# openai/multiagent-particle-envs

Measured on AMD Instinct MI355X. Metric: env steps/sec (whole node), simple_spread N=3, batch=65536 per GPU, higher is better.
Workload: dtype f32; 1 GPU; simple_spread A=3 L=3, 65536 worlds/GPU, fresh one-hot moves, reset every 25 steps; steps commanded to the step server; protocol=fresh, step-server (one doorbell per episode), batch_per_gpu=65536, global_batch=65536, mode=step-server, commands=auto, barrier_backend=none

## Files before the change

### multiagent_particle_envs_amd/csrc/mpe_split.hip

```cpp
#include <type_traits>

#include "mpe_internal.h"

#ifndef MPE_SPLIT_ABLATE
#define MPE_SPLIT_ABLATE 0
#endif

#ifdef MPE_PHASE_CLOCK
#define MPE_STAMP(k)                                                                                              \
  do {                                                                                                            \
    if (blockIdx.x < 4 && lane == 0 && b.force && t < 32)                                                         \
      reinterpret_cast<unsigned long long *>(b.force)[(((size_t)blockIdx.x * 16 + role) * 32 + t) * 8 + (k)] =     \
          __builtin_amdgcn_s_memtime();                                                                           \
  } while (0)
#else
#define MPE_STAMP(k) do { } while (0)
#endif

#ifdef MPE_DEVICE_SPAN
#define MPE_SPAN_BEGIN() const unsigned long long span_t0_ = (unsigned long long)wall_clock64()
#define MPE_SPAN_END()                                                                                             \
  do {                                                                                                             \
    if (b_in.force && (threadIdx.x & 63) == 0 && (threadIdx.x >> 6) < 8) {                                           \
      const uintptr_t sp_ = reinterpret_cast<uintptr_t>(b_in.force);                                                \
      if (sp_ & 1) asm volatile("s_waitcnt vmcnt(0) lgkmcnt(0)" ::: "memory");                                      \
      ulonglong2 st_;                                                                                              \
      st_.x = span_t0_;                                                                                            \
      st_.y = (unsigned long long)wall_clock64();                                                                  \
      reinterpret_cast<ulonglong2 *>(sp_ & ~(uintptr_t)7)[(size_t)blockIdx.x * 8 + (threadIdx.x >> 6)] = st_;       \
    }                                                                                                              \
  } while (0)
#else
#define MPE_SPAN_BEGIN() do { } while (0)
#define MPE_SPAN_END() do { } while (0)
#endif

namespace mpe {

#ifndef MPE_SPLIT_DUAL
#define MPE_SPLIT_DUAL 1
#endif
#ifndef MPE_SPLIT_DUAL_OWN_DRAW
#define MPE_SPLIT_DUAL_OWN_DRAW (1 << MPE_SCN_SPREAD)
#endif
template <int KIND>
constexpr bool dual_own_draw() { return ((MPE_SPLIT_DUAL_OWN_DRAW) >> KIND) & 1; }

template <int KIND>
constexpr bool dual_kind() {
  return (MPE_SPLIT_DUAL) &&
         (KIND == MPE_SCN_SIMPLE || KIND == MPE_SCN_SPREAD || KIND == MPE_SCN_TAG || KIND == MPE_SCN_ADVERSARY || KIND == MPE_SCN_PUSH);
}

template <int KIND, int A, int L, int NADV>
struct SplitShape {
  static constexpr int E = A + L;
  static constexpr int XW = KIND == MPE_SCN_SPREAD ? 4 + L
                            : (KIND == MPE_SCN_SIMPLE || KIND == MPE_SCN_ADVERSARY || KIND == MPE_SCN_PUSH ||
                               KIND == MPE_SCN_SPEAKER_LISTENER || KIND == MPE_SCN_REFERENCE) ? 5
                            : KIND == MPE_SCN_WORLD_COMM ? 6 : 4;
  static constexpr int DC = KIND == MPE_SCN_SPEAKER_LISTENER ? 3 : KIND == MPE_SCN_REFERENCE ? 10
                            : (KIND == MPE_SCN_CRYPTO || KIND == MPE_SCN_WORLD_COMM) ? 4 : 2;
  static constexpr int NCH = (KIND == MPE_SCN_ADVERSARY || KIND == MPE_SCN_PUSH || KIND == MPE_SCN_SPEAKER_LISTENER) ? 1
                             : (KIND == MPE_SCN_REFERENCE || KIND == MPE_SCN_CRYPTO) ? 2 : 0;
  static constexpr int DMAX = KIND == MPE_SCN_SIMPLE   ? 2 + 2 * L
                              : KIND == MPE_SCN_SPREAD ? 4 + 2 * L + 4 * (A - 1)
                              : KIND == MPE_SCN_TAG    ? 4 + 2 * L + 2 * (A - 1) + 2 * (A - NADV)
                              : KIND == MPE_SCN_ADVERSARY ? 2 + 2 * L + 2 * (A - 1)
                              : KIND == MPE_SCN_PUSH   ? 7 + 5 * L + 2 * (A - 1)
                              : KIND == MPE_SCN_SPEAKER_LISTENER ? 2 + 2 * L + 3
                              : KIND == MPE_SCN_REFERENCE ? 2 + 2 * L + 3 + 10
                              : KIND == MPE_SCN_CRYPTO ? 8
                              : KIND == MPE_SCN_WORLD_COMM ? 4 + 2 * L + 2 * (A - 1) + 2 * (A - NADV) + 2 + 4
                                                       : 1;
  static constexpr int trows(bool roll) { return (KIND == MPE_SCN_WORLD_COMM && roll) ? 32 : kWave; }
  static constexpr int tile_floats(bool roll) { return trows(roll) * (DMAX | 1); }
  static constexpr int waves(bool dual) { return (dual ? 2 * A : A) + 1; }
  static constexpr size_t lds_bytes(bool roll) {
    return sizeof(float) * ((roll ? 2 : 1) * A * XW * kWave + A * tile_floats(roll) + (roll ? 2 * A * kWave : 0));
  }
};

template <int KIND>
constexpr unsigned speakers_of() {
  return KIND == MPE_SCN_SPEAKER_LISTENER ? 0x1u : KIND == MPE_SCN_REFERENCE ? 0x3u : KIND == MPE_SCN_CRYPTO ? 0x7u
         : KIND == MPE_SCN_WORLD_COMM ? 0x1u : 0u;
}
constexpr int kWordRow = 0, kWordDrawn = 1, kWordRowSys = 2;
template <int WM>
struct Word {
  const float *row;
  int id;
  __device__ __forceinline__ float operator[](int c) const {
    if constexpr (WM == kWordDrawn) return c == id ? 1.f : 0.f;
    else if constexpr (WM == kWordRowSys)
      return __builtin_bit_cast(float, __hip_atomic_load(reinterpret_cast<const int *>(row) + c, __ATOMIC_RELAXED, __HIP_MEMORY_SCOPE_SYSTEM));
    else return row[c];
  }
};
template <int DC, int WM>
__device__ __forceinline__ Word<WM> word_of(const MpeBuffers &b, size_t B, size_t w0, unsigned ln, int j, uint64_t seed,
                                            uint64_t gw, uint64_t gt) {
  Word<WM> wd;
  wd.row = WM == kWordDrawn ? nullptr : b.comm + wave_off(((size_t)j * B + w0) * DC) + ln * DC;
  wd.id = WM == kWordDrawn ? comm_draw(seed, gw, gt, j, DC) : 0;
  return wd;
}

template <int KIND, int RP>
constexpr int aux_policy() { return (KIND == MPE_SCN_TAG && RP == kRowsSc1) ? kRowsSc1 : kRowsPlain; }

template <int KIND, int A, int L, int NADV, bool ROLL, int AUX, int WM = (ROLL ? kWordDrawn : kWordRow)>
__device__ __forceinline__ void reward_wave(const NarrowDesc &d, const float *const sz , const MpeBuffers &b, const float *X, int lane,
                                            bool live, unsigned ln, size_t B, size_t w0 ,
                                            size_t ro , uint64_t seed, uint64_t gw,
                                            uint64_t gt, int goal_roll ,
                                            const float (&food_roll)[4] ) {
  constexpr int XW = SplitShape<KIND, A, L, NADV>::XW;
  if (KIND == MPE_SCN_SIMPLE) {
    if (live) {
#pragma unroll
      for (int a = 0; a < A; ++a) {
        if (b.rew) store_aux<AUX>(b.rew + wave_off(ro + (size_t)a * B) + ln, -X[(a * XW + 4) * kWave + lane]);
        if (b.done) store_aux<AUX>(b.done + wave_off(ro + (size_t)a * B) + ln, 0);
      }
    }
  }
  if (KIND == MPE_SCN_SPREAD) {
    if (b.rew || b.info_rew) {
      float px[A], py[A];
#pragma unroll
      for (int a = 0; a < A; ++a) {
        px[a] = X[(a * XW + 0) * kWave + lane];
        py[a] = X[(a * XW + 1) * kWave + lane];
      }
      float lm_term = 0.f, md = 0.f;
      int occupied = 0;
#pragma unroll
      for (int l = 0; l < L; ++l) {
        float m2 = X[(0 * XW + 4 + l) * kWave + lane];
#pragma unroll
        for (int a = 1; a < A; ++a) m2 = fminf(m2, X[(a * XW + 4 + l) * kWave + lane]);
        const float m = fast_sqrt(m2);
        lm_term = lm_term - m;
        md = md + m;
        if (b.info_rew) occupied += sqrt_lt(m2, 0.1f) ? 1 : 0;
      }
      int cnt[A];
#pragma unroll
      for (int a = 0; a < A; ++a) cnt[a] = (sz[a] + sz[a] > 0.f) ? 1 : 0;
#pragma unroll
      for (int a = 0; a < A; ++a) {
#pragma unroll
        for (int c = a + 1; c < A; ++c) {
          const bool hit = sqrt_lt(sq2d(px[a] - px[c], py[a] - py[c]), sz[a] + sz[c]);
          cnt[a] += hit ? 1 : 0;
          cnt[c] += hit ? 1 : 0;
        }
      }
      float r[A];
#pragma unroll
      for (int a = 0; a < A; ++a) {
        const int c = ((d.collide >> a) & 1u) ? cnt[a] : 0;
        cnt[a] = c;
        float ra_ = lm_term;
#pragma unroll
        for (int s = 0; s < A; ++s) ra_ = ra_ - (c > s ? 1.f : 0.f);
        r[a] = ra_;
      }
// ... 157 lines not shown
    for (int g = 0; g < NG; ++g)
#pragma unroll
      for (int v = 0; v < NADV; ++v) {
        const float d2 = sq2d(px[NADV + g] - px[v], py[NADV + g] - py[v]);
        hit[g][v] = sqrt_lt(d2, sz[NADV + g] + sz[v]);
        dmin[v] = fminf(dmin[v], d2);
      }
    float fx[2], fy[2];
#pragma unroll
    for (int f = 0; f < 2; ++f) {
      fx[f] = ROLL ? food_roll[2 * f] : (b.pos + wave_off((size_t)(2 * (A + 1 + f)) * B + w0))[ln];
      fy[f] = ROLL ? food_roll[2 * f + 1] : (b.pos + wave_off((size_t)(2 * (A + 1 + f) + 1) * B + w0))[ln];
    }
    if (live) {
#pragma unroll
      for (int a = 0; a < A; ++a) {
        float r = 0.f;
        if (a < NADV) {
          r = r - 0.1f * fast_sqrt(dmin[a < NADV ? a : 0]);
          if ((d.collide >> a) & 1u) {
#pragma unroll
            for (int g = 0; g < NG; ++g)
#pragma unroll
              for (int v = 0; v < NADV; ++v) r = r + (hit[g][v] ? 5.f : 0.f);
          }
        } else {
          if ((d.collide >> a) & 1u) {
#pragma unroll
            for (int v = 0; v < NADV; ++v) r = r - (hit[a >= NADV ? a - NADV : 0][v] ? 5.f : 0.f);
          }
          r = r - 2.f * tag_bound(fabsf(px[a]));
          r = r - 2.f * tag_bound(fabsf(py[a]));
          float m2 = INFINITY;
#pragma unroll
          for (int f = 0; f < 2; ++f) {
            const float d2 = sq2d(px[a] - fx[f], py[a] - fy[f]);
            r = r + (sqrt_lt(d2, sz[a] + sz[A + 1 + f]) ? 2.f : 0.f);
            m2 = fminf(m2, d2);
          }
          r = r + 0.05f * fast_sqrt(m2);
        }
        const size_t o = ro + (size_t)a * B;
        if (b.rew) store_aux<AUX>(b.rew + wave_off(o) + ln, r);
        if (b.done) store_aux<AUX>(b.done + wave_off(o) + ln, 0);
        if (b.info_collisions) {
          int c = 0;
          if (a < NADV) {
#pragma unroll
            for (int g = 0; g < NG; ++g) c += hit[g][a < NADV ? a : 0] ? 1 : 0;
          }
          store_aux<AUX>(b.info_collisions + wave_off(o) + ln, c);
        }
      }
    }
  }
}

typedef float vf2 __attribute__((ext_vector_type(2)));
typedef __attribute__((address_space(4))) const vf2 cvf2;
__device__ __forceinline__ vf2 pol_act2(vf2 x, bool tnh) { return vf2{pol_act(x.x, tnh), pol_act(x.y, tnh)}; }
template <int NO2>
__device__ __forceinline__ void pol_layer0(const cvf2 *W, const float *row, int sw, int D, float *rec, vf2 (&h)[NO2]) {
#pragma unroll
  for (int j = 0; j < NO2; ++j) h[j] = W[D * NO2 + j];
  for (int k = 0; k < D; ++k) {
    const float x = row[(((k >> 2) ^ sw) << 2) | (k & 3)];
    if (rec) rec[k] = x;
    const vf2 xx = {x, x};
#pragma unroll
    for (int j = 0; j < NO2; ++j) h[j] = __builtin_elementwise_fma(W[k * NO2 + j], xx, h[j]);
  }
}
template <int NO2>
__device__ __forceinline__ void pol_layer(const cvf2 *W, const vf2 (&h)[32], vf2 (&o)[NO2]) {
#pragma unroll
  for (int j = 0; j < NO2; ++j) o[j] = W[64 * NO2 + j];
#pragma unroll
  for (int k = 0; k < 64; ++k) {
    const float x = (k & 1) ? h[k >> 1].y : h[k >> 1].x;
    const vf2 xx = {x, x};
#pragma unroll
    for (int j = 0; j < NO2; ++j) o[j] = __builtin_elementwise_fma(W[k * NO2 + j], xx, o[j]);
    if ((k & 3) == 3) __builtin_amdgcn_sched_barrier(0);
  }
}
__device__ __forceinline__ void pol_logits(const float *Wg, int nl, bool tnh, const float *row, int sw, int D, float *rec,
                                           float (&z)[5]) {
  const cvf2 *W = (const cvf2 *)(uintptr_t)Wg;
  vf2 o[4];
  if (nl == 1) {
    pol_layer0<4>(W, row, sw, D, rec, o);
  } else {
    vf2 h[32];
    pol_layer0<32>(W, row, sw, D, rec, h);
#pragma unroll
    for (int j = 0; j < 32; ++j) h[j] = pol_act2(h[j], tnh);
    const cvf2 *W1 = W + (size_t)(D + 1) * 32;
    if (nl == 2) {
      pol_layer<4>(W1, h, o);
    } else {
      const cvf2 *W2 = W1 + 65 * 32;
#pragma unroll
      for (int j = 0; j < 4; ++j) o[j] = W2[64 * 4 + j];
#pragma unroll 1
      for (int c = 0; c < 4; ++c) {
        vf2 g[8];
#pragma unroll
        for (int j = 0; j < 8; ++j) g[j] = W1[64 * 32 + 8 * c + j];
#pragma unroll
        for (int k = 0; k < 64; ++k) {
          const float x = (k & 1) ? h[k >> 1].y : h[k >> 1].x;
          const vf2 xx = {x, x};
#pragma unroll
          for (int j = 0; j < 8; ++j) g[j] = __builtin_elementwise_fma(W1[k * 32 + 8 * c + j], xx, g[j]);
          if ((k & 7) == 7) __builtin_amdgcn_sched_barrier(0);
        }
#pragma unroll
        for (int u = 0; u < 16; ++u) {
          const float x = pol_act((u & 1) ? g[u >> 1].y : g[u >> 1].x, tnh);
          const vf2 xx = {x, x};
#pragma unroll
          for (int j = 0; j < 4; ++j) o[j] = __builtin_elementwise_fma(W2[(16 * c + u) * 4 + j], xx, o[j]);
        }
      }
    }
  }
  z[0] = o[0].x; z[1] = o[0].y; z[2] = o[1].x; z[3] = o[1].y; z[4] = o[2].x;
}

template <int AUX>
__device__ __forceinline__ void store_state(const MpeBuffers &b, size_t B, int i, size_t w0, unsigned ln, float mx,
                                            float my, float mvx, float mvy) {
  store_aux<AUX>(b.pos + wave_off((size_t)(2 * i) * B + w0) + ln, mx);
  store_aux<AUX>(b.pos + wave_off((size_t)(2 * i + 1) * B + w0) + ln, my);
  store_aux<AUX>(b.vel + wave_off((size_t)(2 * i) * B + w0) + ln, mvx);
  store_aux<AUX>(b.vel + wave_off((size_t)(2 * i + 1) * B + w0) + ln, mvy);
}

struct ServeArgs {
  unsigned long long *door;
  unsigned long long *flag;
  unsigned int *status;
  const float *act_ring;
  const float *comm_ring;
  int32_t ring, slots;
  unsigned long long timeout_ticks;
};
__device__ __forceinline__ unsigned long long door_load(const unsigned long long *p) {
  const unsigned long long v = __hip_atomic_load(p, __ATOMIC_RELAXED, __HIP_MEMORY_SCOPE_SYSTEM);
  const uint32_t lo = __builtin_amdgcn_readfirstlane((uint32_t)v), hi = __builtin_amdgcn_readfirstlane((uint32_t)(v >> 32));
  return ((unsigned long long)hi << 32) | lo;
}
__device__ __forceinline__ void drain_stores() { asm volatile("s_waitcnt vmcnt(0)" ::: "memory"); }

template <int KIND, int A, int L, int NADV, bool ROLL, int RP ,
          bool DUALP = false ,
          bool SERVE = false ,
          bool POL = false >
__device__ __forceinline__ void split_body(float *const g_pos, float *const g_vel, const float *const g_act, const int32_t *const g_ids,
                                           const size_t B, const int g_wpw, const int g_observe_only, const unsigned g_movable,
                                           const NarrowDesc &d, const MpeBuffers &b_in, const RollArgs &ra, const ServeArgs &sv,
                                           const PolArgs &pol) {
  static_assert(!SERVE || (ROLL && RP == kRowsSc1), "the step server: a rollout instantiation, write-through stores");
  static_assert(!POL || (ROLL && !SERVE && !DUALP), "the policy rollout: a single-role rollout instantiation");
  static_assert(!POL || KIND == MPE_SCN_SIMPLE || KIND == MPE_SCN_SPREAD || KIND == MPE_SCN_ADVERSARY || KIND == MPE_SCN_PUSH,
                "the policy rollout: scenarios whose observation rows read no other agent's velocity");
  constexpr int WM = SERVE ? kWordRowSys : (ROLL ? kWordDrawn : kWordRow);
  using S = SplitShape<KIND, A, L, NADV>;
  MPE_SPAN_BEGIN();
  MpeBuffers b = b_in;
  b.pos = g_pos;
  b.vel = g_vel;
  b.act = g_act;
  b.ids = g_ids;
  constexpr int E = A + L, XW = S::XW;
  constexpr int AUX = SERVE ? kRowsSc1 : aux_policy<KIND, RP>();
  extern __shared__ __attribute__((aligned(16))) float smem[];
  const int lane = threadIdx.x & (kWave - 1);
  constexpr bool DUAL = DUALP && ROLL;
  constexpr bool OWN_DRAW = DUAL && dual_own_draw<KIND>();
  constexpr int NAW = DUAL ? 2 * A : A;
  const int role = __builtin_amdgcn_readfirstlane((int)(threadIdx.x >> 6));
  const bool is_agent = role < NAW;
  const bool is_rows = DUAL && role >= A && role < NAW;
  const int i = is_agent ? (role >= A ? role - A : role) : 0;
  const int wpw = g_wpw;
  const size_t w0 = (size_t)blockIdx.x * (size_t)wpw;
  if (w0 >= B) return;
#ifdef MPE_STRESS_DELAY_WAVE
  if (role == (MPE_STRESS_DELAY_WAVE) % A)
    for (int k = 0; k < 10; ++k) __builtin_amdgcn_s_sleep(127);
#endif
  const int nvalid = (B - w0) < (size_t)wpw ? (int)(B - w0) : wpw;
  const bool live = lane < nvalid;
  const unsigned ln = (unsigned)(live ? lane : nvalid - 1) & 63u;
  const size_t w = w0 + (size_t)ln;
  float *const xch = smem;
  float *const tile = smem + (ROLL ? 2 : 1) * A * XW * kWave + i * S::tile_floats(ROLL);
  int *const mv = reinterpret_cast<int *>(smem + (ROLL ? 2 : 1) * A * XW * kWave + A * S::tile_floats(ROLL));

  const int T = ROLL ? ra.T : 1;
  const size_t obs_stride = (ra.trajectory || SERVE) ? (size_t)d.obs_off[A] * B : 0;
  const size_t row_stride = (ra.trajectory || SERVE) ? (size_t)A * B : 0;
  int blk0 = 0, mvt0 = 0;
  unsigned long long seen = 0;
  int *const idle_cnt = reinterpret_cast<int *>(smem + SplitShape<KIND, A, L, NADV>::lds_bytes(true) / sizeof(float));
  if constexpr (SERVE) {
    blk0 = (int)(ra.step0 % (uint64_t)sv.slots);
    mvt0 = (int)(ra.step0 % (uint64_t)sv.ring);
    if (threadIdx.x < 3) idle_cnt[threadIdx.x] = 0;
    __syncthreads();
  }
  auto block_of = [&](const int t) { return SERVE ? (blk0 + t) % sv.slots : t; };
  auto with_words = [&](const int t) {
    MpeBuffers q = b;
    if constexpr (SERVE)
      q.comm = sv.comm_ring ? sv.comm_ring + (size_t)((mvt0 + t) % sv.ring) * ((size_t)A * B * SplitShape<KIND, A, L, NADV>::DC) : nullptr;
    return q;
  };
  auto wait_door = [&](const int t, const bool publisher) -> bool {
    if constexpr (!SERVE) return true;
    const unsigned long long g = ra.step0 + (unsigned long long)t;
    if (seen > g) return true;
    seen = door_load(sv.door);
    if (seen > g) return true;
    drain_stores();
    bool told = t == 0;
    if (!publisher && !told && lane == 0) __hip_atomic_fetch_add(&idle_cnt[t & 1], 1, __ATOMIC_RELEASE, __HIP_MEMORY_SCOPE_WORKGROUP);
    const unsigned long long t_begin = (unsigned long long)wall_clock64();
    for (;;) {
      if (publisher && !told) {
        const int n = __builtin_amdgcn_readfirstlane(__hip_atomic_load(&idle_cnt[t & 1], __ATOMIC_ACQUIRE, __HIP_MEMORY_SCOPE_WORKGROUP));
        if (n >= NAW) {
          if (lane == 0) __hip_atomic_store(sv.flag + blockIdx.x, g, __ATOMIC_RELAXED, __HIP_MEMORY_SCOPE_SYSTEM);
          told = true;
        }
      }
      __builtin_amdgcn_s_sleep(4);
      seen = door_load(sv.door);
      if (seen > g) return true;
      if ((unsigned long long)wall_clock64() - t_begin > sv.timeout_ticks) {
        if (lane == 0) {
          __hip_atomic_store(sv.status, 1u, __ATOMIC_RELAXED, __HIP_MEMORY_SCOPE_SYSTEM);
          __hip_atomic_store(&idle_cnt[2], 1, __ATOMIC_RELAXED, __HIP_MEMORY_SCOPE_WORKGROUP);
        }
        return false;
      }
    }
  };
  auto next_commanded = [&](const int t) -> bool {
    if constexpr (!SERVE) return false;
    return t + 1 < T && seen > ra.step0 + (unsigned long long)t + 1;
  };
  auto aborted = [&]() -> bool {
    if constexpr (!SERVE) return false;
    return __builtin_amdgcn_readfirstlane(__hip_atomic_load(&idle_cnt[2], __ATOMIC_RELAXED, __HIP_MEMORY_SCOPE_WORKGROUP)) != 0;
  };

  if (!is_agent) {
    constexpr bool TRACK = ROLL && (KIND == MPE_SCN_CRYPTO || KIND == MPE_SCN_WORLD_COMM);
    const uint64_t gw_r = ra.world_offset + w;
    int goal_r = (ROLL && KIND == MPE_SCN_CRYPTO) ? (b.choice + wave_off(w0))[ln] : 0;
    float food[4] = {0.f, 0.f, 0.f, 0.f};
    if (ROLL && KIND == MPE_SCN_WORLD_COMM) {
#pragma unroll
      for (int f = 0; f < 2; ++f) {
        food[2 * f] = (b.pos + wave_off((size_t)(2 * (A + 1 + f)) * B + w0))[ln];
        food[2 * f + 1] = (b.pos + wave_off((size_t)(2 * (A + 1 + f) + 1) * B + w0))[ln];
      }
    }
    float sz[E];
#pragma unroll
    for (int e = 0; e < E; ++e) sz[e] = d.size[e];
    pin_s(sz);
    int cd = -1;
    uint64_t ep_r = 0;
    if (TRACK && ra.episode_len > 0) {
      const uint64_t len = (uint64_t)ra.episode_len, r = ra.step0 % len;
      cd = r == 0 ? 0 : (int)(len - r);
      ep_r = ra.step0 / len + (r ? 1 : 0);
    }
    for (int t = 0; t < T; ++t) {
      MPE_STAMP(0);
      if (SERVE && !wait_door(t, true)) {
        __syncthreads();
        return;
      }
      if (TRACK && cd >= 0) {
        if (cd == 0) {
          if (KIND == MPE_SCN_CRYPTO) goal_r = choice_draw(ra.seed, gw_r, ep_r, 0, d.choice_pop[0]);
          if (KIND == MPE_SCN_WORLD_COMM) {
#pragma unroll
            for (int f = 0; f < 2; ++f) reset_draw(ra.seed, gw_r, ep_r, A + 1 + f, ra.landmark_range, food[2 * f], food[2 * f + 1]);
          }
          ++ep_r;
          cd = ra.episode_len - 1;
        } else {
          --cd;
        }
      }
      if (ROLL && !SERVE && !OWN_DRAW && !POL && t + 1 < T) {
        const uint64_t gt1 = ra.step0 + (uint64_t)t + 1;
#pragma unroll
        for (int q = 0; q < (A + 3) / 4; ++q) {
          const U4 o = action_block(ra.seed, gw_r, gt1, q);
          const uint32_t word[4] = {o.x, o.y, o.z, o.w};
#pragma unroll
          for (int k = 0; k < 4; ++k)
            if (4 * q + k < A) mv[(((t + 1) & 1) * A + 4 * q + k) * kWave + lane] = move_of(word[k]);
        }
      }
      const float *const X = xch + (ROLL ? (t & 1) * A * XW * kWave : 0);
      MPE_STAMP(1);
      if (SERVE) drain_stores();
      __syncthreads();
      if (SERVE) {
        if (t > 0 && lane == 0) __hip_atomic_store(sv.flag + blockIdx.x, ra.step0 + (unsigned long long)t, __ATOMIC_RELAXED, __HIP_MEMORY_SCOPE_SYSTEM);
        if (lane == 0) idle_cnt[t & 1] = 0;
        if (aborted()) return;
      }
      MPE_STAMP(2);
      if (!(MPE_SPLIT_ABLATE & 2))
      reward_wave<KIND, A, L, NADV, ROLL, AUX, WM>(d, sz, with_words(t), X, lane, live, ln, B, w0, (size_t)block_of(t) * row_stride + w0,
                                                   ra.seed, gw_r, ra.step0 + (uint64_t)t, goal_r, food);
      MPE_STAMP(3);
    }
    if (SERVE) {
      drain_stores();
      __syncthreads();
      if (lane == 0) __hip_atomic_store(sv.flag + blockIdx.x, ra.step0 + (unsigned long long)T, __ATOMIC_RELAXED, __HIP_MEMORY_SCOPE_SYSTEM);
    }
    MPE_SPAN_END();
    return;
  }

  float px[E], py[E];
#pragma unroll
  for (int e = 0; e < E; ++e) {
    px[e] = (b.pos + wave_off((size_t)(2 * e) * B + w0))[ln];
    py[e] = (b.pos + wave_off((size_t)(2 * e + 1) * B + w0))[ln];
  }
  float mvx = (b.vel + wave_off((size_t)(2 * i) * B + w0))[ln];
  float mvy = (b.vel + wave_off((size_t)(2 * i + 1) * B + w0))[ln];
  const bool movable_i = (g_movable >> i) & 1u;
  const bool step_world = ROLL || !g_observe_only;
  float ux0 = 0.f, uy0 = 0.f;
  if (!ROLL && step_world && movable_i && (b.act || b.ids)) fetch_action_wave(b, B, i, w0, ln, 1.0f, ux0, uy0);

  float kc[9 + E];
  kc[0] = d.size[i]; kc[1] = d.inv_mass[i]; kc[2] = d.accel[i]; kc[3] = d.max_speed[i];
  kc[4] = d.dt; kc[5] = d.damp; kc[6] = d.cforce; kc[7] = d.cmargin; kc[8] = d.cmargin_inv;
#pragma unroll
  for (int e = 0; e < E; ++e) kc[9 + e] = d.size[e];
  pin_s(kc);
  const float size_i = kc[0], mass_i = kc[1], accel_i = kc[2], maxspd_i = kc[3];
  const float k_dt = kc[4], k_damp = kc[5], k_cforce = kc[6], k_cmargin = kc[7], k_cmargin_inv = kc[8];
  const float *const size_e = kc + 9;
  const int obs_off_i = d.obs_off[i];
  const bool collide_i = (d.collide >> i) & 1u;
  float mx = 0.f, my = 0.f;
#pragma unroll
  for (int a = 0; a < A; ++a)
    if (a == i) { mx = px[a]; my = py[a]; }

  const uint64_t gw = ra.world_offset + w;
  constexpr bool HAS_GOAL = KIND == MPE_SCN_ADVERSARY || KIND == MPE_SCN_PUSH;
  constexpr int NCH = S::NCH, DC = S::DC;
  int goal = NCH >= 1 ? (b.choice + wave_off(w0))[ln] : 0;
  int pick1 = NCH >= 2 ? (b.choice + wave_off(B + w0))[ln] : 0;

  int countdown = -1;
  uint64_t ep = 0;
  if (ROLL && ra.episode_len > 0) {
    const uint64_t len = (uint64_t)ra.episode_len, r = ra.step0 % len;
    countdown = r == 0 ? 0 : (int)(len - r);
    ep = ra.step0 / len + (r ? 1 : 0);
  }

  float gx = 0.f, gy = 0.f;
  [[maybe_unused]] bool did_reset = false;
  auto roll_reset = [&]() -> bool {
    const bool reset_now = countdown == 0;
    if (countdown >= 0) countdown = reset_now ? ra.episode_len - 1 : countdown - 1;
    if (reset_now) {
#pragma unroll
      for (int e = 0; e < E; ++e) reset_draw(ra.seed, gw, ep, e, e < A ? 1.0f : ra.landmark_range, px[e], py[e]);
#pragma unroll
      for (int a = 0; a < A; ++a)
        if (a == i) { mx = px[a]; my = py[a]; }
      mvx = 0.f;
      mvy = 0.f;
      if (NCH >= 1) goal = choice_draw(ra.seed, gw, ep, 0, d.choice_pop[0]);
      if (NCH >= 2) pick1 = choice_draw(ra.seed, gw, ep, 1, d.choice_pop[1]);
      ++ep;
      if (SERVE) did_reset = true;
    }
    return reset_now;
  };
  [[maybe_unused]] float pa1 = 0.f, pa2 = 0.f, pa3 = 0.f, pa4 = 0.f;
  auto step_forces = [&](const int t, float &fx, float &fy) {
    float ux, uy;
    const uint64_t gt = ra.step0 + (uint64_t)t;
    if (ROLL) {
      if constexpr (!POL) roll_reset();
      if constexpr (SERVE) {
        const float *const mt = sv.act_ring + (size_t)((mvt0 + t) % sv.ring) * ((size_t)A * B * MPE_ACTION_DIM);
        typedef float vf4 __attribute__((ext_vector_type(4)));
        const float *const mp = mt + wave_off(((size_t)i * B + w0) * MPE_ACTION_DIM) + (ln * MPE_ACTION_DIM + 1);
        vf4 m4;
        asm volatile("global_load_dwordx4 %0, %1, off sc0 sc1\n\ts_waitcnt vmcnt(0)" : "=&v"(m4) : "v"(mp) : "memory");
        if (movable_i) {
          ux = (m4.x - m4.y) * accel_i;
          uy = (m4.z - m4.w) * accel_i;
        } else {
          ux = 0.f;
          uy = 0.f;
        }
      } else if constexpr (POL) {
        ux = (pa1 - pa2) * accel_i;
        uy = (pa3 - pa4) * accel_i;
      } else {
      const int m = (t == 0 || OWN_DRAW) ? action_draw(ra.seed, gw, gt, i) : mv[((t & 1) * A + i) * kWave + lane];
      ux = ((m == 1 ? 1.f : 0.f) - (m == 2 ? 1.f : 0.f)) * accel_i;
      uy = ((m == 3 ? 1.f : 0.f) - (m == 4 ? 1.f : 0.f)) * accel_i;
      }
    } else if (step_world && movable_i) {
      if (b.act || b.ids) { ux = ux0 * accel_i; uy = uy0 * accel_i; }
      else fetch_action_wave(b, B, i, w0, ln, accel_i, ux, uy);
    } else {
      ux = 0.f;
      uy = 0.f;
    }
    fx = ux + 0.f;
    fy = uy + 0.f;
    if (movable_i && step_world && collide_i && !(MPE_SPLIT_ABLATE & 1)) {
#pragma unroll
      for (int j = 0; j < E; ++j) {
        if (j == i) continue;
        if (!((d.collide >> j) & 1u)) continue;
        float cx, cy;
        contact_force(mx - px[j], my - py[j], size_i + size_e[j], k_cforce, k_cmargin, k_cmargin_inv, cx, cy);
        fx = cx + fx;
        fy = cy + fy;
      }
    }
  };
  auto step_integrate = [&](const int t, const float fx, const float fy) {
    if (movable_i && step_world) {
      integrate_one(mx, my, mvx, mvy, fx, fy, mass_i, maxspd_i, k_damp, k_dt);
#ifdef MPE_STRESS_STORE_BEFORE_BARRIER
      if (live && (!ROLL || t == T - 1)) store_state<AUX>(b, B, i, w0, ln, mx, my, mvx, mvy);
#endif
    }
#ifdef MPE_PHASE_CLOCK
    asm volatile("" ::"v"(mx), "v"(my), "v"(mvx), "v"(mvy));
#endif
  };
  auto publish = [&](const int t) {
    float *const X = xch + (ROLL ? (t & 1) * A * XW * kWave : 0);
    X[(i * XW + 0) * kWave + lane] = mx;
    X[(i * XW + 1) * kWave + lane] = my;
    X[(i * XW + 2) * kWave + lane] = mvx;
    X[(i * XW + 3) * kWave + lane] = mvy;
    if (KIND == MPE_SCN_SPREAD) {
#pragma unroll
      for (int l = 0; l < L; ++l) X[(i * XW + 4 + l) * kWave + lane] = sq2d(mx - px[A + l], my - py[A + l]);
    }
    if (KIND == MPE_SCN_SIMPLE) X[(i * XW + 4) * kWave + lane] = sq2d(mx - px[A], my - py[A]);
    if (HAS_GOAL || KIND == MPE_SCN_SPEAKER_LISTENER) {
      goal_pos<A, L>(px, py, goal, gx, gy);
      X[(i * XW + 4) * kWave + lane] = sq2d(mx - gx, my - gy);
    }
    if constexpr (KIND == MPE_SCN_REFERENCE) {
      goal_pos<A, L>(px, py, i == 0 ? pick1 : goal, gx, gy);
      X[(i * XW + 4) * kWave + lane] = sq2d(mx - gx, my - gy);
    }
    if constexpr (KIND == MPE_SCN_WORLD_COMM) {
#pragma unroll
      for (int f = 0; f < 2; ++f)
        X[(i * XW + 4 + f) * kWave + lane] =
            sqrt_lt(sq2d(mx - px[A + 3 + f], my - py[A + 3 + f]), size_i + size_e[A + 3 + f]) ? 1.f : -1.f;
    }
  };
  auto behind_barrier = [&](const int t) {
#ifndef MPE_STRESS_STORE_BEFORE_BARRIER
    if (movable_i && step_world && live && (!ROLL || (SERVE ? !next_commanded(t) : t == T - 1)) && !(MPE_SPLIT_ABLATE & 8))
      store_state<AUX>(b, B, i, w0, ln, mx, my, mvx, mvy);
#endif
    if constexpr (SERVE) {
      if (did_reset && live) {
#pragma unroll
        for (int l = 0; l < L; ++l)
          if (l % A == i) {
            store_aux<AUX>(b.pos + wave_off((size_t)(2 * (A + l)) * B + w0) + ln, px[A + l]);
            store_aux<AUX>(b.pos + wave_off((size_t)(2 * (A + l) + 1) * B + w0) + ln, py[A + l]);
          }
        if (NCH >= 1 && i == 0) {
          store_aux<AUX>(b.choice + wave_off(w0) + ln, goal);
          if (NCH >= 2) store_aux<AUX>(b.choice + wave_off(B + w0) + ln, pick1);
        }
        if (!movable_i) store_state<AUX>(b, B, i, w0, ln, mx, my, mvx, mvy);
      }
      did_reset = false;
    }
    if constexpr (KIND == MPE_SCN_ADVERSARY && !ROLL) {
      if (live && b.info_rew) {
        store_aux<AUX>(b.info_rew + wave_off((size_t)i * B + w0) + ln, sq2d(mx - gx, my - gy));
        if (b.info_min_dists) {
#pragma unroll
          for (int l = 0; l < L; ++l)
            store_aux<AUX>(b.info_min_dists + wave_off(((size_t)l * A + i) * B + w0) + ln, sq2d(mx - px[A + l], my - py[A + l]));
        }
      }
    }
    const float *const X = xch + (ROLL ? (t & 1) * A * XW * kWave : 0);
#pragma unroll
    for (int a = 0; a < A; ++a) {
      if (a == i) { px[a] = mx; py[a] = my; continue; }
      px[a] = X[(a * XW + 0) * kWave + lane];
      py[a] = X[(a * XW + 1) * kWave + lane];
    }
#ifdef MPE_PHASE_CLOCK
#pragma unroll
    for (int a = 0; a < A; ++a) asm volatile("" ::"v"(px[a]), "v"(py[a]));
#endif
  };
  [[maybe_unused]] int pol_D = 0, pol_S = 0, pol_sw = 0;
  auto note_tile = [&](auto dc, auto pc) {
    if constexpr (POL) {
      constexpr int D = decltype(dc)::value;
      constexpr bool P = decltype(pc)::value;
      constexpr int NS = (P && row_vec4<D>()) ? D / 4 : 0;
      pol_D = D;
      pol_S = P ? pair_stride<D>() : tile_stride<D>();
      pol_sw = NS ? swz4<NS>(lane) : 0;
    }
  };
  auto rows = [&](const int t, const bool pre) {
    if (MPE_SPLIT_ABLATE & 4) return;
    const float *const X = xch + (ROLL ? (t & 1) * A * XW * kWave : 0);
    const uint64_t gt = ra.step0 + (uint64_t)t;
    float *const obs_t = b.obs + (size_t)block_of(t) * obs_stride;
    [[maybe_unused]] const MpeBuffers bw = with_words(t);
    if (KIND == MPE_SCN_SIMPLE) {
      constexpr int D = 2 + 2 * L;
      {
        RowPairs<D> r(tile, lane);
        r.put(0, mvx, mvy);
#pragma unroll
        for (int l = 0; l < L; ++l) r.put(2 + 2 * l, px[A + l] - mx, py[A + l] - my);
      }
      note_tile(std::integral_constant<int, D>{}, std::bool_constant<true>{});
        if (!pre) flush_rows<D, true, RP>(tile, obs_t + B * obs_off_i + w0 * D, nvalid, lane, d.vec4);
    }
    if (KIND == MPE_SCN_SPREAD) {
      constexpr int D = 4 + 2 * L + 4 * (A - 1);
      {
        RowPairs<D> r(tile, lane);
        r.put(0, mvx, mvy);
        r.put(2, mx, my);
#pragma unroll
        for (int l = 0; l < L; ++l) r.put(4 + 2 * l, px[A + l] - mx, py[A + l] - my);
        int k = 4 + 2 * L;
#pragma unroll
        for (int j = 0; j < A; ++j) {
          if (j == i) continue;
// ... 423 lines not shown
  split_body<KIND, A, L, NADV, ROLL, RP, DUALP, SERVE, false>(g_pos, g_vel, g_act, g_ids, B, g_wpw, g_observe_only, g_movable, d, b_in,
                                                              ra, sv, PolArgs{});
}
template <int KIND, int A, int L, int NADV>
__global__ void __launch_bounds__((SplitShape<KIND, A, L, NADV>::waves(false) * kWave))
k_split_policy(float *const g_pos, float *const g_vel, const float *const g_act, const int32_t *const g_ids, const size_t B,
               const int g_wpw, const int g_observe_only, const unsigned g_movable, const NarrowDesc d, const MpeBuffers b_in,
               const RollArgs ra, const PolArgs pol) {
  split_body<KIND, A, L, NADV, true, kRowsNt, false, false, true>(g_pos, g_vel, g_act, g_ids, B, g_wpw, g_observe_only, g_movable, d,
                                                                  b_in, ra, ServeArgs{}, pol);
}


constexpr size_t kRowsNtFromBytes = 8u << 20, kRollNtFromBytes = 12u << 20;
using SplitFn = void (*)(float *, float *, const float *, const int32_t *, const size_t, const int, const int, const unsigned,
                         const NarrowDesc, const MpeBuffers, const RollArgs, const ServeArgs);
struct SplitEntry {
  int kind, A, L, nadv;
  SplitFn step, step_small, roll, roll_small;
  SplitFn roll_dual, roll_dual_small;
  SplitFn serve, serve_dual;
  size_t lds_step, lds_roll;
};
template <int KIND, int A, int L, int NADV>
constexpr SplitFn serve_fn() { return k_split<KIND, A, L, NADV, true, kRowsSc1, false, true>; }
template <int KIND, int A, int L, int NADV>
constexpr SplitFn serve_dual_fn() {
  if constexpr (dual_kind<KIND>() && SplitShape<KIND, A, L, NADV>::waves(true) * kWave <= 1024)
    return k_split<KIND, A, L, NADV, true, kRowsSc1, true, true>;
  else return nullptr;
}
template <int KIND, int A, int L, int NADV, int RP>
constexpr SplitFn dual_fn() {
  if constexpr (dual_kind<KIND>() && SplitShape<KIND, A, L, NADV>::waves(true) * kWave <= 1024) return k_split<KIND, A, L, NADV, true, RP, true>;
  else return nullptr;
}
#define MPE_SPLIT_ENTRY(KIND, A, L, NADV)                                                                         \
  { KIND, A, L, NADV, k_split<KIND, A, L, NADV, false, kRowsNt>, k_split<KIND, A, L, NADV, false, kRowsSc1>,       \
    k_split<KIND, A, L, NADV, true, kRowsNt>, k_split<KIND, A, L, NADV, true, kRowsSc1>,                           \
    dual_fn<KIND, A, L, NADV, kRowsNt>(), dual_fn<KIND, A, L, NADV, kRowsSc1>(), serve_fn<KIND, A, L, NADV>(),     \
    serve_dual_fn<KIND, A, L, NADV>(),                                                                             \
    SplitShape<KIND, A, L, NADV>::lds_bytes(false), SplitShape<KIND, A, L, NADV>::lds_bytes(true) }

static const SplitEntry kSplitTable[] = {
    MPE_SPLIT_ENTRY(MPE_SCN_SIMPLE, 1, 1, 0),
    MPE_SPLIT_ENTRY(MPE_SCN_SPREAD, 1, 1, 0), MPE_SPLIT_ENTRY(MPE_SCN_SPREAD, 2, 2, 0),
    MPE_SPLIT_ENTRY(MPE_SCN_SPREAD, 3, 3, 0), MPE_SPLIT_ENTRY(MPE_SCN_SPREAD, 4, 4, 0),
    MPE_SPLIT_ENTRY(MPE_SCN_SPREAD, 5, 5, 0), MPE_SPLIT_ENTRY(MPE_SCN_SPREAD, 6, 6, 0),
    MPE_SPLIT_ENTRY(MPE_SCN_TAG, 4, 2, 3), MPE_SPLIT_ENTRY(MPE_SCN_TAG, 2, 1, 1),
    MPE_SPLIT_ENTRY(MPE_SCN_TAG, 6, 3, 4),
    MPE_SPLIT_ENTRY(MPE_SCN_ADVERSARY, 3, 2, 1), MPE_SPLIT_ENTRY(MPE_SCN_PUSH, 2, 2, 1),
    MPE_SPLIT_ENTRY(MPE_SCN_SPEAKER_LISTENER, 2, 3, 0), MPE_SPLIT_ENTRY(MPE_SCN_REFERENCE, 2, 3, 0),
    MPE_SPLIT_ENTRY(MPE_SCN_CRYPTO, 3, 2, 1), MPE_SPLIT_ENTRY(MPE_SCN_WORLD_COMM, 6, 5, 4),
#ifdef MPE_SPLIT_TEAM_GRID
    MPE_SPLIT_ENTRY(MPE_SCN_ADVERSARY, 2, 1, 1), MPE_SPLIT_ENTRY(MPE_SCN_ADVERSARY, 3, 2, 2),
    MPE_SPLIT_ENTRY(MPE_SCN_ADVERSARY, 4, 3, 1), MPE_SPLIT_ENTRY(MPE_SCN_ADVERSARY, 4, 3, 2),
    MPE_SPLIT_ENTRY(MPE_SCN_ADVERSARY, 5, 4, 1), MPE_SPLIT_ENTRY(MPE_SCN_ADVERSARY, 5, 4, 2),
    MPE_SPLIT_ENTRY(MPE_SCN_ADVERSARY, 6, 5, 1), MPE_SPLIT_ENTRY(MPE_SCN_ADVERSARY, 6, 5, 2),
    MPE_SPLIT_ENTRY(MPE_SCN_WORLD_COMM, 3, 5, 2), MPE_SPLIT_ENTRY(MPE_SCN_WORLD_COMM, 4, 5, 3),
    MPE_SPLIT_ENTRY(MPE_SCN_WORLD_COMM, 5, 5, 4), MPE_SPLIT_ENTRY(MPE_SCN_WORLD_COMM, 6, 5, 5),
    MPE_SPLIT_ENTRY(MPE_SCN_WORLD_COMM, 4, 5, 2), MPE_SPLIT_ENTRY(MPE_SCN_WORLD_COMM, 5, 5, 3),
    MPE_SPLIT_ENTRY(MPE_SCN_WORLD_COMM, 7, 5, 5),
    MPE_SPLIT_ENTRY(MPE_SCN_WORLD_COMM, 5, 5, 2), MPE_SPLIT_ENTRY(MPE_SCN_WORLD_COMM, 6, 5, 3),
    MPE_SPLIT_ENTRY(MPE_SCN_WORLD_COMM, 7, 5, 4), MPE_SPLIT_ENTRY(MPE_SCN_WORLD_COMM, 8, 5, 5),
#endif
};

static const SplitEntry *find_split(int kind, int A, int L, int nadv) {
  for (const SplitEntry &e : kSplitTable)
    if (e.kind == kind && e.A == A && e.L == L && (kind < MPE_SCN_TAG || e.nadv == nadv)) return &e;
  return nullptr;
}

bool split_supports(int kind, int A, int L, int nadv) { return find_split(kind, A, L, nadv) != nullptr; }

int launch_split(bool roll, int kind, int A, int L, int nadv, const NarrowDesc &d, const MpeBuffers &b, size_t B,
                 const RollArgs &ra, hipStream_t stream) {
  const SplitEntry *e = find_split(kind, A, L, nadv);
  if (!e) return MPE_EUNSUPPORTED;
  RollArgs r2 = ra;
#ifdef MPE_SPLIT_WPW
  r2.wpw = MPE_SPLIT_WPW;
#else
  r2.wpw = kWave;
#endif
  const unsigned grid = (unsigned)((B + r2.wpw - 1) / r2.wpw);
  const size_t row_bytes = (size_t)d.obs_off[A] * sizeof(float) * B;
  const bool small = row_bytes < (roll ? kRollNtFromBytes : kRowsNtFromBytes);
  SplitFn fn = roll ? (small ? e->roll_small : e->roll) : small ? e->step_small : e->step;
  int waves = A + 1;
  static const int n_cu = [] {
    int dev = 0, v = 0;
    if (hipGetDevice(&dev) == hipSuccess && hipDeviceGetAttribute(&v, hipDeviceAttributeMultiprocessorCount, dev) == hipSuccess && v > 0) return v;
    (void)hipGetLastError();
    return 256;
  }();
#ifdef MPE_SPLIT_DUAL_MAX_WG_PER_CU_X2
  const unsigned dual_max = (unsigned)n_cu * (MPE_SPLIT_DUAL_MAX_WG_PER_CU_X2) / 2;
#else
  const unsigned dual_max = (unsigned)n_cu * 3 / 2;
#endif
  SplitFn dual = small ? e->roll_dual_small : e->roll_dual;
  if (roll && dual && grid <= dual_max) {
    fn = dual;
    waves = 2 * A + 1;
  }
  hipLaunchKernelGGL(fn, dim3(grid), dim3(waves * kWave), roll ? e->lds_roll : e->lds_step, stream,
                     b.pos, b.vel, b.act, b.ids, B, (int)r2.wpw, (int)r2.observe_only, (unsigned)d.movable, d, b, r2, ServeArgs{});
  return (int)hipGetLastError();
}

using PolicyFn = void (*)(float *, float *, const float *, const int32_t *, const size_t, const int, const int, const unsigned,
                         const NarrowDesc, const MpeBuffers, const RollArgs, const PolArgs);
struct PolicyEntry {
  int kind, A, L, nadv;
  PolicyFn fn;
  size_t lds;
};
#define MPE_POLICY_ENTRY(KIND, A, L, NADV) \
  { KIND, A, L, NADV, k_split_policy<KIND, A, L, NADV>, SplitShape<KIND, A, L, NADV>::lds_bytes(true) }
static const PolicyEntry kPolicyTable[] = {
    MPE_POLICY_ENTRY(MPE_SCN_SIMPLE, 1, 1, 0),
    MPE_POLICY_ENTRY(MPE_SCN_SPREAD, 1, 1, 0), MPE_POLICY_ENTRY(MPE_SCN_SPREAD, 2, 2, 0), MPE_POLICY_ENTRY(MPE_SCN_SPREAD, 3, 3, 0),
    MPE_POLICY_ENTRY(MPE_SCN_ADVERSARY, 3, 2, 1), MPE_POLICY_ENTRY(MPE_SCN_PUSH, 2, 2, 1),
};
static const PolicyEntry *find_policy(int kind, int A, int L, int nadv) {
  for (const PolicyEntry &e : kPolicyTable)
    if (e.kind == kind && e.A == A && e.L == L && (kind < MPE_SCN_TAG || e.nadv == nadv)) return &e;
  return nullptr;
}
bool split_policy_supports(int kind, int A, int L, int nadv) { return find_policy(kind, A, L, nadv) != nullptr; }
int launch_split_policy(int kind, int A, int L, int nadv, const NarrowDesc &d, const MpeBuffers &b, size_t B, const RollArgs &ra,
                        const PolArgs &pol, hipStream_t stream) {
  const PolicyEntry *e = find_policy(kind, A, L, nadv);
  if (!e) return MPE_EUNSUPPORTED;
  RollArgs r2 = ra;
  r2.wpw = kWave;
  const unsigned grid = (unsigned)((B + kWave - 1) / kWave);
  if (e->lds > 64 * 1024) {
    const hipError_t rc = hipFuncSetAttribute(reinterpret_cast<const void *>(e->fn), hipFuncAttributeMaxDynamicSharedMemorySize, (int)e->lds);
    if (rc != hipSuccess) return (int)rc;
  }
  hipLaunchKernelGGL(e->fn, dim3(grid), dim3((A + 1) * kWave), e->lds, stream, b.pos, b.vel, b.act, b.ids, B, (int)r2.wpw, 0,
                     (unsigned)d.movable, d, b, r2, pol);
  return (int)hipGetLastError();
}

bool serve_supports(int kind, int A, int L, int nadv) {
  const SplitEntry *e = find_split(kind, A, L, nadv);
  return e && e->serve;
}
unsigned serve_grid(size_t B) { return (unsigned)((B + kWave - 1) / kWave); }

int launch_split_serve(int kind, int A, int L, int nadv, const NarrowDesc &d, const MpeBuffers &b, size_t B, const RollArgs &ra,
                       const ServeHandles &h, hipStream_t stream) {
  const SplitEntry *e = find_split(kind, A, L, nadv);
  if (!e || !e->serve) return MPE_EUNSUPPORTED;
  RollArgs r2 = ra;
  r2.wpw = kWave;
  ServeArgs sv;
  sv.door = reinterpret_cast<unsigned long long *>(h.door);
  sv.flag = reinterpret_cast<unsigned long long *>(h.flag);
  sv.status = h.status;
  sv.act_ring = h.act_ring;
  sv.comm_ring = h.comm_ring;
  sv.ring = h.ring;
  sv.slots = h.slots;
  sv.timeout_ticks = h.timeout_ticks;
  const size_t lds = e->lds_roll + 16;
  const unsigned grid = serve_grid(B);
  int per_cu = 0, dev = 0, n_cu = 0;
  if (hipGetDevice(&dev) != hipSuccess || hipDeviceGetAttribute(&n_cu, hipDeviceAttributeMultiprocessorCount, dev) != hipSuccess) {
    (void)hipGetLastError();
    return MPE_EUNSUPPORTED;
  }
  SplitFn fn = e->serve;
  int waves = A + 1;
#ifndef MPE_SERVE_NO_DUAL
  if (e->serve_dual && grid <= (unsigned)n_cu * 3 / 2) {
    fn = e->serve_dual;
    waves = 2 * A + 1;
  }
#endif
  if (hipOccupancyMaxActiveBlocksPerMultiprocessor(&per_cu, reinterpret_cast<const void *>(fn), waves * kWave, lds) != hipSuccess) {
    (void)hipGetLastError();
    return MPE_EUNSUPPORTED;
  }
  if (!h.ahead && (size_t)grid > (size_t)n_cu * (size_t)(per_cu > 1 ? per_cu - 1 : per_cu)) return MPE_ESERVER_TOO_LARGE;
  hipLaunchKernelGGL(fn, dim3(grid), dim3(waves * kWave), lds, stream, b.pos, b.vel, b.act, b.ids, B, (int)r2.wpw, 0,
                     (unsigned)d.movable, d, b, r2, sv);
  return (int)hipGetLastError();
}

__global__ void k_serve_ring(unsigned long long *const door, const unsigned long long n) {
  if (threadIdx.x == 0 && blockIdx.x == 0) __hip_atomic_fetch_add(door, n, __ATOMIC_RELAXED, __HIP_MEMORY_SCOPE_SYSTEM);
}
__global__ void __launch_bounds__(256)
k_serve_wait(const unsigned long long *const flag, const unsigned n_flags, const unsigned long long completed,
             unsigned int *const status, const unsigned long long timeout_ticks) {
  const unsigned k = blockIdx.x * blockDim.x + threadIdx.x;
  if (k >= n_flags) return;
  const unsigned long long t0 = (unsigned long long)wall_clock64();
  while (__hip_atomic_load(flag + k, __ATOMIC_RELAXED, __HIP_MEMORY_SCOPE_SYSTEM) < completed) {
    __builtin_amdgcn_s_sleep(8);
    if ((unsigned long long)wall_clock64() - t0 > timeout_ticks) {
      __hip_atomic_store(status, 2u, __ATOMIC_RELAXED, __HIP_MEMORY_SCOPE_SYSTEM);
      return;
    }
  }
}
int launch_serve_ring(uint64_t *door, uint64_t n, hipStream_t stream) {
  hipLaunchKernelGGL(k_serve_ring, dim3(1), dim3(64), 0, stream, reinterpret_cast<unsigned long long *>(door), (unsigned long long)n);
  return (int)hipGetLastError();
}
int launch_serve_wait(const uint64_t *flag, unsigned n_flags, uint64_t completed, uint32_t *status, uint64_t timeout_ticks,
                      hipStream_t stream) {
  hipLaunchKernelGGL(k_serve_wait, dim3((n_flags + 255) / 256), dim3(256), 0, stream, reinterpret_cast<const unsigned long long *>(flag),
                     n_flags, (unsigned long long)completed, status, (unsigned long long)timeout_ticks);
  return (int)hipGetLastError();
}

}
```

Baseline: 19.12 billion env-steps/s.

## Batch step-server move fetches across several ring slots and cache occupancy queries

After: 19.14 billion env-steps/s (median of 2 runs). Within noise of the previous version (+0.1%).

```diff
diff --git a/multiagent_particle_envs_amd/csrc/mpe_split.hip b/multiagent_particle_envs_amd/csrc/mpe_split.hip
--- a/multiagent_particle_envs_amd/csrc/mpe_split.hip
+++ b/multiagent_particle_envs_amd/csrc/mpe_split.hip
@@ -1,4 +1,7 @@
+#include <map>
+#include <mutex>
 #include <type_traits>
+#include <utility>
 
 #include "mpe_internal.h"
 
@@ -13,8 +16,14 @@
       reinterpret_cast<unsigned long long *>(b.force)[(((size_t)blockIdx.x * 16 + role) * 32 + t) * 8 + (k)] =     \
           __builtin_amdgcn_s_memtime();                                                                           \
   } while (0)
+#define MPE_STAMP_AT(k, clk)                                                                                        \
+  do {                                                                                                            \
+    if (blockIdx.x < 4 && lane == 0 && b.force && t < 32)                                                         \
+      reinterpret_cast<unsigned long long *>(b.force)[(((size_t)blockIdx.x * 16 + role) * 32 + t) * 8 + (k)] = (clk); \
+  } while (0)
 #else
 #define MPE_STAMP(k) do { } while (0)
+#define MPE_STAMP_AT(k, clk) do { } while (0)
 #endif
 
 #ifdef MPE_DEVICE_SPAN
@@ -478,6 +487,45 @@
   return ((unsigned long long)hi << 32) | lo;
 }
 __device__ __forceinline__ void drain_stores() { asm volatile("s_waitcnt vmcnt(0)" ::: "memory"); }
+
+constexpr int kMoveBatch = 4;
+template <int KIND, int A, int L, int NADV, bool DUALP>
+constexpr int move_batch() {
+#ifdef MPE_MOVE_BATCH
+  return MPE_MOVE_BATCH;
+#else
+  if (DUALP) return KIND == MPE_SCN_TAG && A == 4 ? 3 : kMoveBatch;
+  if (dual_kind<KIND>()) return 1;
+  return KIND == MPE_SCN_CRYPTO ? 1 : KIND == MPE_SCN_SPEAKER_LISTENER ? 2 : kMoveBatch;
+#endif
+}
+constexpr int kMoveBatchMax = 5;
+typedef float move_f4 __attribute__((ext_vector_type(4)));
+template <int N>
+__device__ __forceinline__ void load_move_rows(move_f4 (&m)[kMoveBatchMax], const float *const (&p)[kMoveBatchMax], const unsigned off) {
+  static_assert(N >= 1 && N <= kMoveBatchMax, "rows per fetch");
+  if constexpr (N == 1) {
+    const float *const p0 = reinterpret_cast<const float *>(reinterpret_cast<const char *>(p[0]) + off);
+    asm volatile("global_load_dwordx4 %0, %1, off sc0 sc1\n\ts_waitcnt vmcnt(0)" : "=&v"(m[0]) : "v"(p0) : "memory");
+  }
+  if constexpr (N == 2)
+    asm volatile("s_nop 4\n\tglobal_load_dwordx4 %0, %2, %3 sc0 sc1\n\tglobal_load_dwordx4 %1, %2, %4 sc0 sc1\n\ts_waitcnt vmcnt(0)"
+                 : "=&v"(m[0]), "=&v"(m[1]) : "v"(off), "s"(p[0]), "s"(p[1]) : "memory");
+  if constexpr (N == 3)
+    asm volatile("s_nop 4\n\tglobal_load_dwordx4 %0, %3, %4 sc0 sc1\n\tglobal_load_dwordx4 %1, %3, %5 sc0 sc1\n\t"
+                 "global_load_dwordx4 %2, %3, %6 sc0 sc1\n\ts_waitcnt vmcnt(0)"
+                 : "=&v"(m[0]), "=&v"(m[1]), "=&v"(m[2]) : "v"(off), "s"(p[0]), "s"(p[1]), "s"(p[2]) : "memory");
+  if constexpr (N == 4)
+    asm volatile("s_nop 4\n\tglobal_load_dwordx4 %0, %4, %5 sc0 sc1\n\tglobal_load_dwordx4 %1, %4, %6 sc0 sc1\n\t"
+                 "global_load_dwordx4 %2, %4, %7 sc0 sc1\n\tglobal_load_dwordx4 %3, %4, %8 sc0 sc1\n\ts_waitcnt vmcnt(0)"
+                 : "=&v"(m[0]), "=&v"(m[1]), "=&v"(m[2]), "=&v"(m[3]) : "v"(off), "s"(p[0]), "s"(p[1]), "s"(p[2]), "s"(p[3]) : "memory");
+  if constexpr (N == 5)
+    asm volatile("s_nop 4\n\tglobal_load_dwordx4 %0, %5, %6 sc0 sc1\n\tglobal_load_dwordx4 %1, %5, %7 sc0 sc1\n\t"
+                 "global_load_dwordx4 %2, %5, %8 sc0 sc1\n\tglobal_load_dwordx4 %3, %5, %9 sc0 sc1\n\t"
+                 "global_load_dwordx4 %4, %5, %10 sc0 sc1\n\ts_waitcnt vmcnt(0)"
+                 : "=&v"(m[0]), "=&v"(m[1]), "=&v"(m[2]), "=&v"(m[3]), "=&v"(m[4])
+                 : "v"(off), "s"(p[0]), "s"(p[1]), "s"(p[2]), "s"(p[3]), "s"(p[4]) : "memory");
+}
 
 template <int KIND, int A, int L, int NADV, bool ROLL, int RP ,
           bool DUALP = false ,
@@ -724,20 +772,63 @@
     return reset_now;
   };
   [[maybe_unused]] float pa1 = 0.f, pa2 = 0.f, pa3 = 0.f, pa4 = 0.f;
+  constexpr int KB = SERVE ? move_batch<KIND, A, L, NADV, DUALP>() : 1, KQ = KB > 1 ? KB - 1 : 1;
+  static_assert(KB >= 1 && KB <= kMoveBatchMax, "kMoveBatch");
+  [[maybe_unused]] float qx[KQ], qy[KQ];
+  [[maybe_unused]] int qn = 0;
   auto step_forces = [&](const int t, float &fx, float &fy) {
     float ux, uy;
     const uint64_t gt = ra.step0 + (uint64_t)t;
     if (ROLL) {
       if constexpr (!POL) roll_reset();
       if constexpr (SERVE) {
-        const float *const mt = sv.act_ring + (size_t)((mvt0 + t) % sv.ring) * ((size_t)A * B * MPE_ACTION_DIM);
-        typedef float vf4 __attribute__((ext_vector_type(4)));
-        const float *const mp = mt + wave_off(((size_t)i * B + w0) * MPE_ACTION_DIM) + (ln * MPE_ACTION_DIM + 1);
-        vf4 m4;
-        asm volatile("global_load_dwordx4 %0, %1, off sc0 sc1\n\ts_waitcnt vmcnt(0)" : "=&v"(m4) : "v"(mp) : "memory");
+        float dx, dy;
+#ifdef MPE_PHASE_CLOCK
+        const unsigned long long clk_move = __builtin_amdgcn_s_memtime();
+#endif
+        if (KB > 1 && qn > 0) {
+          dx = qx[0];
+          dy = qy[0];
+#pragma unroll
+          for (int j = 0; j + 1 < KQ; ++j) { qx[j] = qx[j + 1]; qy[j] = qy[j + 1]; }
+          --qn;
+        } else {
+          const unsigned long long ahead = seen - gt;
+          const int left = T - t;
+          const int cmd = ahead < (unsigned long long)KB ? (int)ahead : KB;
+          const int n = KB > 1 ? __builtin_amdgcn_readfirstlane(cmd < left ? cmd : left) : 1;
+          const size_t tensor = (size_t)A * B * MPE_ACTION_DIM;
+          const float *const row = sv.act_ring + wave_off(((size_t)i * B + w0) * MPE_ACTION_DIM);
+          const unsigned off = (ln * MPE_ACTION_DIM + 1) * (unsigned)sizeof(float);
+          const float *mp[kMoveBatchMax];
+          move_f4 m4[kMoveBatchMax];
+          int slot = (mvt0 + t) % sv.ring;
+#pragma unroll
+          for (int j = 0; j < kMoveBatchMax; ++j) {
+            mp[j] = row + wave_off((size_t)slot * tensor);
+            slot = slot + 1 == sv.ring ? 0 : slot + 1;
+          }
+          if (KB >= 5 && n == 5) load_move_rows<5>(m4, mp, off);
+          else if (KB >= 4 && n == 4) load_move_rows<4>(m4, mp, off);
+          else if (KB >= 3 && n == 3) load_move_rows<3>(m4, mp, off);
+          else if (KB >= 2 && n == 2) load_move_rows<2>(m4, mp, off);
+          else load_move_rows<1>(m4, mp, off);
+          dx = m4[0].x - m4[0].y;
+          dy = m4[0].z - m4[0].w;
+          if constexpr (KB > 1) {
+#pragma unroll
+            for (int j = 0; j < KQ; ++j)
+              if (j + 1 < n) { qx[j] = m4[j + 1].x - m4[j + 1].y; qy[j] = m4[j + 1].z - m4[j + 1].w; }
+            qn = n - 1;
+          }
+        }
+#ifdef MPE_PHASE_CLOCK
+        MPE_STAMP_AT(6, clk_move);
+        MPE_STAMP_AT(7, __builtin_amdgcn_s_memtime());
+#endif
         if (movable_i) {
-          ux = (m4.x - m4.y) * accel_i;
-          uy = (m4.z - m4.w) * accel_i;
+          ux = dx * accel_i;
+          uy = dy * accel_i;
         } else {
           ux = 0.f;
           uy = 0.f;
@@ -1467,6 +1558,35 @@
 }
 unsigned serve_grid(size_t B) { return (unsigned)((B + kWave - 1) / kWave); }
 
+constexpr int kServeMaxDevices = 64;
+static std::mutex g_serve_cache_mutex;
+static int serve_cu_count(int dev) {
+  static int n_cu[kServeMaxDevices];
+  std::lock_guard<std::mutex> hold(g_serve_cache_mutex);
+  if (dev >= 0 && dev < kServeMaxDevices && n_cu[dev] > 0) return n_cu[dev];
+  int v = 0;
+  if (hipDeviceGetAttribute(&v, hipDeviceAttributeMultiprocessorCount, dev) != hipSuccess || v <= 0) {
+    (void)hipGetLastError();
+    return 0;
+  }
+  if (dev >= 0 && dev < kServeMaxDevices) n_cu[dev] = v;
+  return v;
+}
+static int serve_blocks_per_cu(SplitFn fn, int dev, int threads, size_t lds) {
+  static std::map<std::pair<const void *, int>, int> known;
+  const std::pair<const void *, int> key(reinterpret_cast<const void *>(fn), dev);
+  std::lock_guard<std::mutex> hold(g_serve_cache_mutex);
+  const auto it = known.find(key);
+  if (it != known.end()) return it->second;
+  int per_cu = 0;
+  if (hipOccupancyMaxActiveBlocksPerMultiprocessor(&per_cu, key.first, threads, lds) != hipSuccess || per_cu <= 0) {
+    (void)hipGetLastError();
+    return 0;
+  }
+  known[key] = per_cu;
+  return per_cu;
+}
+
 int launch_split_serve(int kind, int A, int L, int nadv, const NarrowDesc &d, const MpeBuffers &b, size_t B, const RollArgs &ra,
                        const ServeHandles &h, hipStream_t stream) {
   const SplitEntry *e = find_split(kind, A, L, nadv);
@@ -1484,11 +1604,13 @@
   sv.timeout_ticks = h.timeout_ticks;
   const size_t lds = e->lds_roll + 16;
   const unsigned grid = serve_grid(B);
-  int per_cu = 0, dev = 0, n_cu = 0;
-  if (hipGetDevice(&dev) != hipSuccess || hipDeviceGetAttribute(&n_cu, hipDeviceAttributeMultiprocessorCount, dev) != hipSuccess) {
+  int dev = 0;
+  if (hipGetDevice(&dev) != hipSuccess) {
     (void)hipGetLastError();
     return MPE_EUNSUPPORTED;
   }
+  const int n_cu = serve_cu_count(dev);
+  if (n_cu <= 0) return MPE_EUNSUPPORTED;
   SplitFn fn = e->serve;
   int waves = A + 1;
 #ifndef MPE_SERVE_NO_DUAL
@@ -1497,11 +1619,11 @@
     waves = 2 * A + 1;
   }
 #endif
-  if (hipOccupancyMaxActiveBlocksPerMultiprocessor(&per_cu, reinterpret_cast<const void *>(fn), waves * kWave, lds) != hipSuccess) {
-    (void)hipGetLastError();
-    return MPE_EUNSUPPORTED;
-  }
-  if (!h.ahead && (size_t)grid > (size_t)n_cu * (size_t)(per_cu > 1 ? per_cu - 1 : per_cu)) return MPE_ESERVER_TOO_LARGE;
+  if (!h.ahead) {
+    const int per_cu = serve_blocks_per_cu(fn, dev, waves * kWave, lds);
+    if (per_cu <= 0) return MPE_EUNSUPPORTED;
+    if ((size_t)grid > (size_t)n_cu * (size_t)(per_cu > 1 ? per_cu - 1 : per_cu)) return MPE_ESERVER_TOO_LARGE;
+  }
   hipLaunchKernelGGL(fn, dim3(grid), dim3(waves * kWave), lds, stream, b.pos, b.vel, b.act, b.ids, B, (int)r2.wpw, 0,
                      (unsigned)d.movable, d, b, r2, sv);
   return (int)hipGetLastError();
```
